# shenwei356/LexicMap

Measured on AMD Instinct MI355X. Metric: queries/sec (lexicmap search hot path, seed index HBM-resident), higher is better.
Workload: dtype u64

## Files before the change

### lexicmap_amd/csrc/lm_algos.h

```cpp
#pragma once
#include <stdint.h>

#if defined(__HIPCC__)
#define LM_HD __host__ __device__ __forceinline__
#define LM_HDN __host__ __device__ inline
#else
#define LM_HD inline
#define LM_HDN inline
#endif

#define LM_NULL_OFF (-1073741824)

LM_HD int lm_clz64(uint64_t x) {
#if defined(__HIP_DEVICE_COMPILE__)
    return x ? __clzll((long long)x) : 64;
#else
    return x ? __builtin_clzll(x) : 64;
#endif
}

LM_HD uint8_t lm_base2bit(uint8_t c) {
    switch (c | 0x20) {
    case 'c': case 'b': case 's': case 'y': return 1;
    case 'g': case 'k': return 2;
// ... 1258 lines not shown
}
LM_HD bool lm_pa_rule_bit(const uint32_t *rule, uint32_t f, int p) {
    const uint32_t p9 = f >> ((p - LM_PFX_BASES2) << 1);
    return (f & ((1u << ((p - 9) << 1)) - 1u)) == 0 && ((rule[p9 >> 5] >> (p9 & 31)) & 1u) != 0;
}
LM_HD bool lm_pa_candidate3(const uint32_t *bloom, int blog, const uint32_t *rule, const uint32_t *bits11, int log,
                            uint32_t f, int p) {
    const uint32_t p11 = f >> ((p - LM_PFX_BASES) << 1);
    const uint32_t a = lm_pa_bloom_slot(p11, 0, blog), b = lm_pa_bloom_slot(p11, 1, blog);
    bool hit = (((bloom[a >> 5] >> (a & 31)) & (bloom[b >> 5] >> (b & 31))) & 1u) != 0;
    if (hit && log > blog) {
        const uint32_t h = lm_pa_filter_slot(p11, log);
        hit = ((bits11[h >> 5] >> (h & 31)) & 1u) != 0;
    }
    return hit || lm_pa_rule_bit(rule, f, p);
}

LM_HD bool lm_tree_search_range_tab(const uint64_t *keys, int n, uint64_t key, int p, int K, const uint32_t *tab,
                                    int tab_bits, int *lo_out, int *hi_out) {
    if (n <= 0) return false;
    if (p > K) p = K;
    const int sh = (K - p) << 1;
    const uint64_t low = sh >= 64 ? ~0ull : ((1ull << sh) - 1);
    const uint64_t left = key & ~low, right = key | low;
    const uint32_t b = (uint32_t)(key >> ((K << 1) - tab_bits));
    int lo = lm_lower_bound_u64(keys, (int)tab[b], (int)tab[b + 1], left);
    int hi = lm_upper_bound_u64(keys, lo, (int)tab[b + 1], right);
    if (lo < hi) {
        *lo_out = lo;
        *hi_out = hi;
// ... 442 lines not shown
```

### lexicmap_amd/csrc/lm_internal.h

```cpp
#pragma once
#include <hip/hip_runtime.h>

#include <algorithm>
#include <atomic>
#include <chrono>
#include <cstdio>
#include <cstdlib>
#include <map>
#include <memory>
#include <deque>
#include <mutex>
#include <shared_mutex>
#include <stdexcept>
#include <string>
#include <unordered_map>
#include <vector>

#include "../../include/lexicmap_hip.h"
#include "lm_format.h"
#include "lm_kernels.h"

namespace lm {

struct HipError : std::runtime_error {
// ... 381 lines not shown
                   unsigned long long *n_out = nullptr);
void lm_screen_capture(lm_index *ix, hipStream_t st, const uint8_t *d_ascii, const std::vector<int64_t> &src_off,
                       const std::vector<int32_t> &len, const std::vector<int32_t> &reg_off, const std::vector<int32_t> &reg_s,
                       const std::vector<int32_t> &reg_e, uint64_t *d_kmers);
}

#define LM_WFA_CLASSES 5
struct lm_tune {
    int wfa_first_nc[LM_WFA_CLASSES] = {2, 2, 4, 8, 8};
    int wfa_win[LM_WFA_CLASSES] = {0, 0, 1, 0, 1};
    int chain1_wave = 1;
    int pa_filter_roll = 1;
    int pa_seg_by_group = 1;
    int pa_drop_nested = 1;
    int pa_rule_map = 1;
    int wfa_resident_pct = 100;
    int arena_reserve_pct = 90;
    int two_lanes = 1;
    int lookup_flat = 1;
    int wfa_r16 = 1;
    int wfa_serial = 0;
    int no_pipeline = 0;
    lm_tune() {
        if (const char *e = getenv("LM_WFA_FIRST_NC")) {
            int v[LM_WFA_CLASSES];
            if (sscanf(e, "%d,%d,%d,%d,%d", &v[0], &v[1], &v[2], &v[3], &v[4]) == LM_WFA_CLASSES)
                for (int c = 0; c < LM_WFA_CLASSES; c++)
                    if (v[c] == 1 || v[c] == 2 || v[c] == 4 || v[c] == 8 || v[c] == 16) wfa_first_nc[c] = v[c];
        }
        if (const char *e = getenv("LM_WFA_WIN"))
            for (int c = 0; c < LM_WFA_CLASSES && e[c]; c++) wfa_win[c] = e[c] == '1';
        if (const char *e = getenv("LM_WFA_R16")) wfa_r16 = atoi(e) != 0;
        if (const char *e = getenv("LM_LOOKUP_FLAT")) lookup_flat = atoi(e) != 0;
        if (const char *e = getenv("LM_CHAIN1_WAVE")) chain1_wave = atoi(e) != 0;
        if (const char *e = getenv("LM_TWO_LANES")) two_lanes = atoi(e) != 0;
        if (const char *e = getenv("LM_ARENA_RESERVE_PCT")) arena_reserve_pct = std::max(0, std::min(100, atoi(e)));
        if (const char *e = getenv("LM_PA_FILTER_ROLL")) pa_filter_roll = atoi(e) != 0;
        if (const char *e = getenv("LM_PA_DROP_NESTED")) pa_drop_nested = atoi(e) != 0;
        if (const char *e = getenv("LM_PA_RULE_MAP")) pa_rule_map = atoi(e) != 0;
    }
};

struct lm_index {
    lm_tune tune;
    int active_lanes = 1;
    int budget_lanes = 1;
    std::mutex mu;
    HostIndex host;
    lm_options opt;
    int device = 0;
    std::string err;
    DBuf<uint64_t> d_masks, d_pk_keys, d_pk_vals, d_out_kmers, d_out_vals, d_g_bg;
    DBuf<uint32_t> d_part_tab, d_g_keep;
    DBuf<int32_t> d_pfx_first, d_g_len, d_g2local;
// ... 56 lines not shown
```

### lexicmap_amd/csrc/lm_kernels.h

```cpp
#pragma once
#include <hip/hip_runtime.h>
#include <stdint.h>

#include "lm_algos.h"
#include "lm_residency.h"

namespace lm {

struct DevIndexView {
    int K, M, mask_prefix;
    const uint64_t *masks;
    const int32_t *pfx_first;
    int part_bases;
    int P1;
    int key_bits;
    int gid_bits, pos_bits;
    const uint64_t *pk_keys;
    const uint64_t *pk_vals;
    const uint32_t *part_tab;
    const int64_t *md_off;
    const uint64_t *g_bg;
    const uint32_t *g_keep;
    const uint64_t *out_kmers;
    const uint64_t *out_vals;
// ... 83 lines not shown
                       float min_score, int32_t *ntask);
void launch_make_tasks(hipStream_t st, DevIndexView ix, const uint64_t *segA, const int64_t *seg_off, int nseg,
                       const LmSub *subs, const int32_t *chain_off_pool, const int32_t *chain_idx_pool,
                       const int32_t *ntask, const int64_t *task_off, const int64_t *qoff, int ext_len,
                       int32_t *order_scratch, Task *tasks);
void launch_task_wlen(hipStream_t st, const Task *tasks, int64_t ntasks, int32_t *wlen);
void launch_task_set_woff(hipStream_t st, Task *tasks, int64_t ntasks, const int64_t *woff);
void launch_extract_windows(hipStream_t st, DevIndexView ix, const Task *tasks, const TaskSrc *src, int64_t ntasks,
                            const int32_t *only, uint8_t *wbuf);
void launch_extract_windows_at(hipStream_t st, DevIndexView ix, const Task *tasks, const TaskSrc *src, const int32_t *idx,
                               const int64_t *dest, int64_t n, uint8_t *wbuf);
void launch_stage_genome_bits(hipStream_t st, const StageCmd *cmds, int64_t n);
void launch_build_cmp_tab(hipStream_t st, const uint64_t *keys_cmp, const int64_t *posoff, const int32_t *nvalid, int nq,
                          int K, const int64_t *tab_off, const int32_t *tab_bits, int64_t tab_words, uint32_t *tab);
void launch_sum_i32(hipStream_t st, const int32_t *v, int64_t n, unsigned long long *out);
void launch_build_cmp_bits(hipStream_t st, const uint64_t *keys_cmp, const int64_t *posoff, const int32_t *nvalid, int nq,
                           int K, const int64_t *bits_off, const int32_t *bits_log, uint32_t *bits);
#define LM_PA_MAX_SEGS 8192
#define LM_PA_RANGE_SEGS 16
#define LM_PA_GROUP 64
void launch_pa_filter(hipStream_t st, DevIndexView ix, const Task *tasks, const TaskSrc *src, int64_t ntasks, const uint8_t *wbuf,
                      const int64_t *posoff, const int32_t *nvalid, const uint32_t *cmp_bits, const int64_t *bits_off,
                      const int32_t *bits_log, int K, int min_prefix, unsigned long long *seg_count, int nseg, int64_t seg_cap,
                      uint64_t *cand, unsigned long long *group_counter, int ncu, int seg_by_group, bool roll = true,
                      bool rule = true);
void launch_pa_search(hipStream_t st, DevIndexView ix, const Task *tasks, const TaskSrc *src, const uint8_t *wbuf, const uint64_t *keys_cmp,
                      const uint32_t *vals_cmp, const int64_t *posoff, const int32_t *nvalid, const uint32_t *cmp_tab,
                      const int64_t *tab_off, const int32_t *tab_bits, int K, int min_prefix,
                      const unsigned long long *seg_count, int nseg, int64_t seg_cap, const uint64_t *cand,
                      unsigned long long *count, int64_t cap, uint64_t *outA, uint64_t *outB, int qbits, int tbits,
                      int xcd_map, bool drop_nested = true);
void launch_pa_task_off_sorted(hipStream_t st, const uint64_t *sortedA, int shift, int64_t total, int64_t ntasks,
                               int64_t *pa_off);
void launch_pa_chain(hipStream_t st, const uint64_t *B, const int64_t *pa_off, int64_t ntasks, int K, LmChain2Opt opt,
                     LmSub *subs, uint8_t *marks, uint64_t *msi, int32_t *stack, LmChain2 *out, int32_t *out_n,
                     int32_t *clr_n, int qbits, int tbits);
void launch_gather_chain2(hipStream_t st, const LmChain2 *in, const int64_t *pa_off, const int32_t *out_n,
                          const int64_t *res_off, int64_t ntasks, LmChain2 *out);
void launch_extend_count(hipStream_t st, const HspIn *hsps, int64_t n, const uint8_t *qseq, const int64_t *qoff,
                         const uint8_t *wbuf, int32_t *cap);
// ... 17 lines not shown
```

### lexicmap_amd/csrc/lm_kernels.hip

```cpp
#include <hip/hip_runtime.h>
#include <stdint.h>

#include <algorithm>

#include "lm_algos.h"
#include "lm_kernels.h"
#include "lm_lookup_dev.h"

namespace lm {

#define LDS_WAVE_SYNC()                                        \
    do {                                                       \
        __builtin_amdgcn_fence(__ATOMIC_RELEASE, "wavefront"); \
        __builtin_amdgcn_wave_barrier();                       \
        __builtin_amdgcn_fence(__ATOMIC_ACQUIRE, "wavefront"); \
    } while (0)

__device__ __forceinline__ int find_segment(const int64_t *off, int n, int64_t x) {
    int lo = 0, hi = n;
    while (lo < hi) {
        int mid = (lo + hi + 1) >> 1;
        if (off[mid] <= x)
            lo = mid;
        else
// ... 62 lines not shown
    for (int64_t t = (int64_t)blockIdx.x * blockDim.x + threadIdx.x; t < total; t += (int64_t)gridDim.x * blockDim.x) {
        const int q = find_segment(tab_off, nq, t);
        const int bits = tab_bits[q], nb = 1 << bits;
        const int b = (int)(t - tab_off[q]);
        const uint64_t *keys = keys_cmp + 2 * posoff[q];
        int n = nvalid[q];
        int lo = n;
        if (b < nb) {
            uint64_t target = (uint64_t)b << ((K << 1) - bits);
            lo = lm_lower_bound_u64(keys, 0, n, target);
        }
        tab[t] = (uint32_t)lo;
    }
}
__global__ __launch_bounds__(256) void k_build_cmp_bits(const uint64_t *__restrict__ keys_cmp,
                                                         const int64_t *__restrict__ posoff,
                                                         const int32_t *__restrict__ nvalid, int nq, int K,
                                                         const int64_t *__restrict__ bits_off,
                                                         const int32_t *__restrict__ bits_log, uint32_t *__restrict__ bits) {
    for (int q = blockIdx.x; q < nq; q += gridDim.x) {
        const uint64_t *keys = keys_cmp + 2 * posoff[q];
        const int n = nvalid[q];
        const int log = bits_log[q];
        uint32_t *b = bits + bits_off[q];
        lm_pa_filter_preset(log, (int)threadIdx.x, (int)blockDim.x, [&](uint64_t w, uint32_t m) { atomicOr(&b[w], m); });
        for (int j = threadIdx.x; j < n; j += blockDim.x)
            lm_pa_filter_set(keys[j], K, log, [&](uint64_t w, uint32_t m) { atomicOr(&b[w], m); });
    }
}

__global__ void k_fill_u32(uint32_t *p, int64_t n, uint32_t v) {
    for (int64_t i = (int64_t)blockIdx.x * blockDim.x + threadIdx.x; i < n; i += (int64_t)gridDim.x * blockDim.x) p[i] = v;
}

__global__ void k_mask(const uint64_t *__restrict__ keys_all, const int64_t *__restrict__ posoff, int nq, int M, int K,
                       const uint64_t *__restrict__ masks, uint64_t *__restrict__ out_kmers,
                       int64_t *__restrict__ out_lo, int64_t *__restrict__ out_hi, uint32_t *__restrict__ first_mask) {
    int64_t total = (int64_t)nq * M;
    for (int64_t t = (int64_t)blockIdx.x * blockDim.x + threadIdx.x; t < total; t += (int64_t)gridDim.x * blockDim.x) {
        int q = (int)(t / M), m = (int)(t % M);
        int64_t base = 2 * posoff[q];
        int n = (int)(2 * (posoff[q + 1] - posoff[q]));
// ... 816 lines not shown
        r = any;
    }
    return r;
}
template <bool ROLL, bool SRC, bool RULE>
__global__ __launch_bounds__(PA_THREADS) void k_pa_filter(DevIndexView ix, const Task *__restrict__ tasks,
                                                           const TaskSrc *__restrict__ src, int64_t ntasks,
                                                           const uint8_t *__restrict__ wbuf,
                                                           const int64_t *__restrict__ posoff,
                                                           const int32_t *__restrict__ nvalid,
                                                           const uint32_t *__restrict__ cmp_bits,
                                                           const int64_t *__restrict__ bits_off,
                                                           const int32_t *__restrict__ bits_log, int K, int min_prefix,
                                                           unsigned long long *__restrict__ seg_count, int nseg,
                                                           int64_t seg_cap, uint64_t *__restrict__ cand,
                                                           unsigned long long *__restrict__ group_counter, int seg_by_group) {
    extern __shared__ uint64_t pa_lds[];
    uint64_t *s_stage = pa_lds;
    uint32_t *s_bloom = (uint32_t *)(pa_lds + PA_WAVES * PA_STAGE);
    uint32_t *s_map9 = s_bloom + (1 << (LM_PA_BLOOM_LOG_MAX - 5));
    uint64_t *s_pend_rec = (uint64_t *)(s_map9 + (1 << (LM_PA_MAP9_LOG - 5)));
    uint32_t *s_pend_pf = (uint32_t *)(s_pend_rec + PA_WAVES * PA_PEND);
    const int tid = threadIdx.x, lane = tid & 63, wave = tid >> 6;
    uint64_t *stg = s_stage + wave * PA_STAGE;
    int n_stg = 0;
    const uint64_t lt_mask = lane ? (~0ull >> (64 - lane)) : 0ull;
    int seg = (int)(((int64_t)blockIdx.x * PA_WAVES + wave) % nseg);
    uint64_t *seg_list = cand + (int64_t)seg * seg_cap;
    auto flush = [&]() {
        if (n_stg == 0) return;
        unsigned long long base = 0;
// ... 3 lines not shown
            if ((int64_t)(base + (unsigned long long)j) < seg_cap) seg_list[base + (unsigned long long)j] = stg[j];
        n_stg = 0;
    };
    auto push = [&](bool c, uint64_t rec) {
        const uint64_t m = __ballot(c);
        if (m == 0) return;
        if (c) stg[n_stg + __popcll(m & lt_mask)] = rec;
        n_stg += __popcll(m);
        if (n_stg > PA_STAGE - 128) flush();
    };
    uint32_t *pend_pf = s_pend_pf + wave * PA_PEND;
    uint64_t *pend_rec = s_pend_rec + wave * PA_PEND;
    int n_pend = 0;
    const uint32_t *cur_qbits = nullptr;
    int cur_log = 0, cur_blog = 0;
    auto pend_round = [&](int cnt) {
        const int idx = n_pend - cnt + lane;
        bool c = false;
        uint64_t rec = 0;
        if (lane < cnt) {
            const uint32_t e = pend_pf[idx];
            rec = pend_rec[idx];
            if constexpr (RULE) {
                const uint32_t h = lm_pa_filter_slot((e & 0x3fffffffu) >> (4 * (int)(e >> 30)), cur_log);
                c = ((cur_qbits[h >> 5] >> (h & 31)) & 1u) != 0;
            } else {
                c = lm_pa_candidate2(s_bloom, cur_blog, s_map9, cur_qbits, cur_log, e & 0x3fffffffu, LM_PFX_BASES + 2 * (int)(e >> 30));
            }
        }
        n_pend -= cnt;
        push(c, rec);
    };
    auto pend = [&](bool c, uint32_t e, uint64_t rec) {
        const uint64_t m = __ballot(c);
        if (m == 0) return;
        if (c) {
            const int slot = n_pend + __popcll(m & lt_mask);
            pend_pf[slot] = e;
            pend_rec[slot] = rec;
        }
// ... 20 lines not shown
    };
    __shared__ int32_t s_q[PA_GROUP], s_rc[PA_GROUP], s_tb[PA_GROUP], s_wlen[PA_GROUP], s_npos[PA_GROUP], s_log[PA_GROUP];
    __shared__ int32_t s_first[PA_GROUP + 1];
    __shared__ int64_t s_goff[PA_GROUP], s_bits[PA_GROUP], s_woff[PA_GROUP];
    __shared__ const uint8_t *s_gb[SRC ? PA_GROUP : 1];
    __shared__ int s_next;
    __shared__ unsigned long long s_grp;
    const int64_t ngroups = (ntasks + PA_GROUP - 1) / PA_GROUP;
    while (true) {
        __syncthreads();
        if (tid == 0) s_grp = atomicAdd(group_counter, 1ull);
        __syncthreads();
        const int64_t grp = (int64_t)s_grp;
        if (grp >= ngroups) break;
        const int64_t t0g = grp * PA_GROUP;
        const int ng = (int)((ntasks < t0g + PA_GROUP ? ntasks : t0g + PA_GROUP) - t0g);
        if (seg_by_group) {
            const int gseg = (int)(grp * (int64_t)(nseg / PA_WAVES) / ngroups) * PA_WAVES + wave;
            if (gseg != seg) {
                flush();
                seg = gseg;
                seg_list = cand + (int64_t)seg * seg_cap;
            }
        }
        __syncthreads();
        if (tid < ng) {
            const Task t = tasks[t0g + tid];
            const int n = nvalid[t.q];
            s_q[tid] = (int32_t)t.q;
            s_rc[tid] = t.rc;
            s_tb[tid] = t.tBegin;
            s_wlen[tid] = t.wlen;
            s_npos[tid] = n > 0 && t.wlen - K + 1 > 0 ? t.wlen - K + 1 : 0;
            if constexpr (SRC) {
                s_gb[tid] = t.g >= 0 ? src[t0g + tid].base : nullptr;
                s_goff[tid] = t.g >= 0 ? src[t0g + tid].off : 0;
            } else {
                s_goff[tid] = t.g >= 0 ? ix.g_off[t.g] : -1;
            }
            s_woff[tid] = t.woff;
            s_bits[tid] = cmp_bits ? bits_off[t.q] : -1;
            s_log[tid] = cmp_bits ? bits_log[t.q] : 0;
        }
        __syncthreads();
        int r0 = 0;
        while (r0 < ng) {
            int r1 = r0 + 1;
            while (r1 < ng && s_q[r1] == s_q[r0]) r1++;
            const int log = s_log[r0], blog = lm_pa_bloom_log(log);
            const uint32_t *qbits = s_bits[r0] >= 0 ? cmp_bits + s_bits[r0] : nullptr;
            cur_qbits = qbits;
            cur_log = log;
            cur_blog = blog;
            if (qbits != nullptr && K >= 16) {
                const uint32_t *gbl = qbits + lm_pa_bloom_word0(log), *g9 = qbits + (RULE ? lm_pa_rule_word0(log) : lm_pa_map9_word0(log));
                const int nb = 1 << (blog - 5);
                for (int j = tid; j < nb; j += PA_THREADS) s_bloom[j] = gbl[j];
// ... 26 lines not shown
                t.tBegin = s_tb[j];
                t.wlen = s_wlen[j];
                const int npos = s_npos[j];
                const int slice = ROLL ? (npos + (s_first[j + 1] - s_first[j]) - 1) / (s_first[j + 1] - s_first[j]) : PA_SLICE;
                const int p0 = (sl - s_first[j]) * slice, p1 = p0 + slice < npos ? p0 + slice : npos;
                const int64_t goff = s_goff[j];
                const uint8_t *gb;
                if constexpr (SRC) gb = s_gb[j];
                else gb = goff >= 0 ? ix.gbits : nullptr;
                const uint8_t *w = wbuf + s_woff[j];
                const int m = pa_min_prefix(min_prefix, t.wlen);
                const int p = m > K ? K : m;
                const bool use_bits = qbits != nullptr && p >= LM_PFX_BASES && K >= LM_PFX_BASES;
                const bool fast_pfx = use_bits && gb != nullptr && p <= 15 && K >= 16;
                const uint64_t rec_t = (uint64_t)(t0g + j) << 32;
                if (ROLL && fast_pfx && K == 31 && p1 > p0) {
                    const int np = p1 - p0;
                    const int bpl = (np + 63) >> 6;
                    const int g0 = t.rc ? t.tBegin + t.wlen - K - (p1 - 1) : t.tBegin + p0;
                    const int64_t abs0 = goff * 4 + g0;
                    const int rl0 = bpl * lane;
                    const int64_t ab = abs0 + (rl0 < np ? rl0 : 0);
                    const uint32_t *gd = (const uint32_t *)gb;
                    const int64_t d0 = ab >> 4, dlast = (abs0 + np + K - 2) >> 4;
                    uint32_t e[5];
#pragma unroll
                    for (int k = 0; k < 5; k++) e[k] = __builtin_bswap32(gd[d0 + k < dlast ? d0 + k : dlast]);
                    const int ob = (int)(ab & 15) * 2;
                    uint32_t S0, S1, S2, S3;
                    {
// ... 23 lines not shown
                            const int r = rl0 + 16 * half + jj;
                            const int i = t.rc ? p1 - 1 - r : p0 + r;
                            const bool in = r < np;
                            bool c0, c1;
                            const uint32_t a0 = pf0 >> sha, a1 = pf1 >> sha;
                            const uint32_t s00 = lm_pa_bloom_slot(a0, 0, blog), s01 = lm_pa_bloom_slot(a0, 1, blog);
                            const uint32_t s10 = lm_pa_bloom_slot(a1, 0, blog), s11 = lm_pa_bloom_slot(a1, 1, blog);
                            const uint32_t b00 = s_bloom[s00 >> 5], b01 = s_bloom[s01 >> 5];
                            const uint32_t b10 = s_bloom[s10 >> 5], b11 = s_bloom[s11 >> 5];
                            const bool h0 = in && (((b00 >> (s00 & 31)) & (b01 >> (s01 & 31))) & 1u) != 0;
                            const bool h1 = in && (((b10 >> (s10 & 31)) & (b11 >> (s11 & 31))) & 1u) != 0;
                            if constexpr (RULE) {
                                const bool r0 = in && lm_pa_rule_bit(s_map9, pf0, p), r1 = in && lm_pa_rule_bit(s_map9, pf1, p);
                                c0 = h0 || r0;
                                c1 = h1 || r1;
                                if (log > blog) {
                                    c0 = r0;
                                    c1 = r1;
                                    pend2(h0 && !r0, h1 && !r1, pf0 | pcode, pf1 | pcode, rec_t | ((uint64_t)(uint32_t)i << 1));
                                }
                            } else {
                                const bool q0 = in && !h0 && (pf0 & m9p) == 0, q1 = in && !h1 && (pf1 & m9p) == 0;
                                c0 = h0;
                                c1 = h1;
                                if (log > blog) {
                                    c0 = c1 = false;
                                    const uint64_t rec = rec_t | ((uint64_t)(uint32_t)i << 1);
                                    pend(h0 || q0, pf0 | pcode, rec);
                                    pend(h1 || q1, pf1 | pcode, rec | 1ull);
                                } else if (__ballot(q0 || q1) != 0ull) {
                                    c0 = pa_partial_rule(q0, c0, pf0, p, blog, s_bloom, s_map9);
// ... 38 lines not shown
                        const bool in = r < np;
                        bool c0, c1;
                        {
                            const uint32_t a0 = pf0 >> ((p - LM_PFX_BASES) << 1), a1 = pf1 >> ((p - LM_PFX_BASES) << 1);
                            const uint32_t s00 = lm_pa_bloom_slot(a0, 0, blog), s01 = lm_pa_bloom_slot(a0, 1, blog);
                            const uint32_t s10 = lm_pa_bloom_slot(a1, 0, blog), s11 = lm_pa_bloom_slot(a1, 1, blog);
                            const uint32_t b00 = s_bloom[s00 >> 5], b01 = s_bloom[s01 >> 5];
                            const uint32_t b10 = s_bloom[s10 >> 5], b11 = s_bloom[s11 >> 5];
                            const bool h0 = in && (((b00 >> (s00 & 31)) & (b01 >> (s01 & 31))) & 1u) != 0;
                            const bool h1 = in && (((b10 >> (s10 & 31)) & (b11 >> (s11 & 31))) & 1u) != 0;
                            if constexpr (RULE) {
                                const bool r0 = in && lm_pa_rule_bit(s_map9, pf0, p), r1 = in && lm_pa_rule_bit(s_map9, pf1, p);
                                const uint32_t pcode = (uint32_t)((p - LM_PFX_BASES) >> 1) << 30;
                                c0 = h0 || r0;
                                c1 = h1 || r1;
                                if (log > blog) {
                                    c0 = r0;
                                    c1 = r1;
                                    pend2(h0 && !r0, h1 && !r1, pf0 | pcode, pf1 | pcode, rec_t | ((uint64_t)(uint32_t)i << 1));
                                }
                            } else {
                                const uint32_t m9p = (1u << ((p - 9) << 1)) - 1u;
                                const bool q0 = in && !h0 && (pf0 & m9p) == 0, q1 = in && !h1 && (pf1 & m9p) == 0;
                                c0 = h0;
                                c1 = h1;
                                if (log > blog) {
                                    c0 = c1 = false;
                                    const uint64_t rec = rec_t | ((uint64_t)(uint32_t)i << 1);
                                    const uint32_t pcode = (uint32_t)((p - LM_PFX_BASES) >> 1) << 30;
                                    pend(h0 || q0, pf0 | pcode, rec);
                                    pend(h1 || q1, pf1 | pcode, rec | 1ull);
// ... 79 lines not shown
        sub = r % blocks_per_seg;
        if (seg >= nseg) return;
    } else {
        seg = blockIdx.x / blocks_per_seg;
        sub = blockIdx.x % blocks_per_seg;
    }
    const uint64_t *cand = cand_all + (int64_t)seg * seg_cap;
    int64_t nc = (int64_t)seg_count[seg];
    if (nc > seg_cap) nc = seg_cap;
    const int sh_t = 2, sh_l = 2 + tbits, sh_q = 8 + tbits, sh_a = 8 + tbits + qbits;
    const uint64_t ccc = lm_ns(1, K), ggg = lm_ns(2, K), ttt = lm_kmer_mask(K);
    const int64_t stride = (int64_t)blocks_per_seg * blockDim.x;
    for (int64_t base = (int64_t)sub * blockDim.x; base < nc; base += stride) {
        const int64_t ci = base + threadIdx.x;
        unsigned long long d_0 = 0, d_1 = 0, d_it = 0, d_an = 0, d_ne = 0;
        if (dbg) d_0 = wall_clock64();
        int j = 0, hi = 0, i = 0;
        int nb = -1, pmin = 0;
        bool rcs = false;
        uint64_t key = 0, right = 0;
        int64_t ti = 0;
        uint32_t qb = 0, qe = 0;
        const uint64_t *keys = nullptr;
        const uint32_t *vals = nullptr;
        if (ci < nc) {
            const uint64_t rec = cand[ci];
            ti = (int64_t)(rec >> 32);
            i = (int)((uint32_t)rec >> 1);
            rcs = (rec & 1ull) != 0;
            const Task t = tasks[ti];
// ... 38 lines not shown
                const uint32_t x = (v & LM_CMP_POS_MASK) >> 1;
                uint32_t pp;
                if (!rcs) {
                    pp = x;
                    if (!((v & 1u) == 1u || pp < qb || pp + lp > qe)) {
                        ok = true;
                        B = lm_pack_anchor((int)pp, (int)lp, i, false, false);
                    }
                } else {
                    pp = x + (uint32_t)K - lp;
                    if (!((v & 1u) == 0u || pp + lp < qb || pp > qe)) {
                        ok = true;
                        B = lm_pack_anchor((int)pp, (int)lp, i + K - (int)lp, true, true);
                    }
                }
                if (ok && lm_pa_nested_match(rcs, K, pmin, (int)lp, nb, v >> LM_CMP_NB_SHIFT, (int)pp, (int)qb)) {
                    if (dbg) d_ne++;
                    if (drop_nested) ok = false;
                }
                j++;
            }
            const uint64_t m = __ballot(ok);
            if (m) {
                if (ok) {
                    if (qbits > 0) {
                        const LmSub u = lm_unpack_anchor(B);
                        B = ((uint64_t)ti << sh_a) | ((uint64_t)(uint32_t)u.qbegin << sh_q) |
                            ((uint64_t)(32 - (int)u.len) << sh_l) | ((uint64_t)(uint32_t)u.tbegin << sh_t) |
                            ((uint64_t)u.qrc << 1) | (uint64_t)u.trc;
                    }
                    const int slot = n_stg + __popcll(m & lt_mask);
                    stg[slot] = B;
                    stt[slot] = (uint32_t)ti;
                }
                n_stg += __popcll(m);
                d_an += (unsigned long long)__popcll(m);
                if (n_stg > PAS_STAGE - 64) flush();
            }
        }
        if (dbg) {
            const unsigned long long nc_w = (unsigned long long)__popcll(__ballot(ci < nc)), d_2 = wall_clock64();
            for (int o = 32; o > 0; o >>= 1) d_ne += __shfl_xor(d_ne, o, 64);
            if (lane == 0) {
                atomicAdd(dbg + 0, nc_w);
                atomicAdd(dbg + 1, 1ull);
                atomicAdd(dbg + 2, d_it);
                atomicAdd(dbg + 3, d_an);
                atomicAdd(dbg + 4, d_1 - d_0);
                atomicAdd(dbg + 5, d_2 - d_1);
                atomicAdd(dbg + 6, d_ne);
            }
        }
    }
    flush();
}
__global__ void k_pa_task_off_sorted(const uint64_t *__restrict__ sortedA, int shift, int64_t total, int64_t ntasks,
                                     int64_t *__restrict__ pa_off) {
    for (int64_t i = (int64_t)blockIdx.x * blockDim.x + threadIdx.x; i <= ntasks; i += (int64_t)gridDim.x * blockDim.x) {
        int64_t lo = 0, hi = total;
        while (lo < hi) {
            int64_t mid = (lo + hi) >> 1;
            if ((sortedA[mid] >> shift) < (uint64_t)i)
                lo = mid + 1;
            else
                hi = mid;
// ... 949 lines not shown
                       n, wbuf);
}
void launch_stage_genome_bits(hipStream_t st, const StageCmd *cmds, int64_t n) {
    if (n <= 0) return;
    hipLaunchKernelGGL(k_stage_genome_bits, dim3((unsigned)std::min<int64_t>(n, 65536)), dim3(256), 0, st, cmds, n);
}
void launch_build_cmp_tab(hipStream_t st, const uint64_t *keys_cmp, const int64_t *posoff, const int32_t *nvalid, int nq,
                          int K, const int64_t *tab_off, const int32_t *tab_bits, int64_t tab_words, uint32_t *tab) {
    LM_LAUNCH_1D(k_build_cmp_tab, tab_words, st, keys_cmp, posoff, nvalid, nq, K, tab_off, tab_bits, tab);
}
void launch_sum_i32(hipStream_t st, const int32_t *v, int64_t n, unsigned long long *out) {
    int g = (int)((n + 255) / 256);
    g = g < 1 ? 1 : (g > 2048 ? 2048 : g);
    hipLaunchKernelGGL(k_sum_i32, dim3(g), dim3(256), 0, st, v, n, out);
}
void launch_build_cmp_bits(hipStream_t st, const uint64_t *keys_cmp, const int64_t *posoff, const int32_t *nvalid, int nq,
                           int K, const int64_t *bits_off, const int32_t *bits_log, uint32_t *bits) {
    int g = nq < 1 ? 1 : (nq > 65536 ? 65536 : nq);
    hipLaunchKernelGGL(k_build_cmp_bits, dim3(g), dim3(256), 0, st, keys_cmp, posoff, nvalid, nq, K, bits_off, bits_log, bits);
}
static decltype(&k_pa_filter<true, true, true>) pa_filter_kernel(bool roll, bool src, bool rule) {
    if (rule) return src ? (roll ? k_pa_filter<true, true, true> : k_pa_filter<false, true, true>) : (roll ? k_pa_filter<true, false, true> : k_pa_filter<false, false, true>);
    return src ? (roll ? k_pa_filter<true, true, false> : k_pa_filter<false, true, false>) : (roll ? k_pa_filter<true, false, false> : k_pa_filter<false, false, false>);
}
void launch_pa_filter(hipStream_t st, DevIndexView ix, const Task *tasks, const TaskSrc *src, int64_t ntasks, const uint8_t *wbuf,
                      const int64_t *posoff, const int32_t *nvalid, const uint32_t *cmp_bits, const int64_t *bits_off,
                      const int32_t *bits_log, int K, int min_prefix, unsigned long long *seg_count, int nseg, int64_t seg_cap,
                      uint64_t *cand, unsigned long long *group_counter, int ncu, int seg_by_group, bool roll, bool rule) {
    const int64_t ngroups = (ntasks + PA_GROUP - 1) / PA_GROUP;
    int g = (int)(ngroups < 1 ? 1 : (ngroups > ncu ? ncu : ngroups));
    static bool lds_set = false;
    if (!lds_set) {
        for (int v = 0; v < 8; v++) (void)hipFuncSetAttribute((const void *)pa_filter_kernel(v & 1, v & 2, v & 4), hipFuncAttributeMaxDynamicSharedMemorySize, PA_LDS_BYTES);
        lds_set = true;
    }
    roll = roll && K == 31;
    auto kern = pa_filter_kernel(roll, src != nullptr, rule);
    hipLaunchKernelGGL(kern, dim3(g), dim3(PA_THREADS), PA_LDS_BYTES, st, ix, tasks, src, ntasks, wbuf,
                       posoff, nvalid, cmp_bits, bits_off, bits_log, K, min_prefix, seg_count, nseg, seg_cap, cand, group_counter,
                       seg_by_group);
}
void launch_pa_search(hipStream_t st, DevIndexView ix, const Task *tasks, const TaskSrc *src, const uint8_t *wbuf, const uint64_t *keys_cmp,
                      const uint32_t *vals_cmp, const int64_t *posoff, const int32_t *nvalid, const uint32_t *cmp_tab,
                      const int64_t *tab_off, const int32_t *tab_bits, int K, int min_prefix,
                      const unsigned long long *seg_count, int nseg, int64_t seg_cap, const uint64_t *cand,
                      unsigned long long *count, int64_t cap, uint64_t *outA, uint64_t *outB, int qbits, int tbits,
                      int xcd_map, bool drop_nested) {
    int bps = xcd_map ? 256 / LM_PA_RANGE_SEGS : (256 * 32 + nseg - 1) / nseg;
    const int64_t need = (seg_cap + 255) / 256;
    if (bps > need) bps = (int)(need < 1 ? 1 : need);
    const int nseg8 = xcd_map ? (nseg / LM_PA_RANGE_SEGS + 7) / 8 * 8 * LM_PA_RANGE_SEGS : nseg;
    static const bool ps_dbg = getenv("LM_DEBUG_PA_SEARCH") != nullptr;
    static unsigned long long *d_dbg = nullptr;
    if (ps_dbg && !d_dbg && hipMalloc((void **)&d_dbg, 8 * sizeof(unsigned long long)) != hipSuccess) d_dbg = nullptr;
    if (ps_dbg && d_dbg) (void)hipMemsetAsync(d_dbg, 0, 8 * sizeof(unsigned long long), st);
    hipLaunchKernelGGL(src ? k_pa_search<true> : k_pa_search<false>, dim3(nseg8 * bps), dim3(256), 0, st, ix, tasks, src, wbuf, keys_cmp, vals_cmp, posoff, nvalid, cmp_tab,
                       tab_off, tab_bits, K, min_prefix, seg_count, seg_cap, bps, cand, count, cap, outA, outB, qbits, tbits, nseg,
                       xcd_map, drop_nested ? 1 : 0, ps_dbg ? d_dbg : nullptr);
    if (ps_dbg && d_dbg) {
        unsigned long long h[8] = {0};
        (void)hipStreamSynchronize(st);
        (void)hipMemcpy(h, d_dbg, sizeof h, hipMemcpyDeviceToHost);
        const unsigned long long found = h[3] + (drop_nested ? h[6] : 0ull);
        fprintf(stderr, "[lm] k_pa_search: %llu candidates in %llu wavefront passes (%.1f per pass), %llu enumeration passes, %llu anchors (%.2f per enumeration pass), wavefront-ms: search %.1f, enumeration %.1f; %llu anchors found, %llu nested in their neighbour's (%.1f %%, %s)\n",
                h[0], h[1], h[1] ? (double)h[0] / (double)h[1] : 0.0, h[2], h[3], h[2] ? (double)h[3] / (double)h[2] : 0.0, (double)h[4] / 1e5, (double)h[5] / 1e5,
                found, h[6], found ? 100.0 * (double)h[6] / (double)found : 0.0, drop_nested ? "not emitted" : "emitted");
    }
}
void launch_pa_task_off_sorted(hipStream_t st, const uint64_t *sortedA, int shift, int64_t total, int64_t ntasks,
                               int64_t *pa_off) {
    LM_LAUNCH_1D(k_pa_task_off_sorted, ntasks + 1, st, sortedA, shift, total, ntasks, pa_off);
}
void launch_pa_chain(hipStream_t st, const uint64_t *B, const int64_t *pa_off, int64_t ntasks, int K, LmChain2Opt opt,
                     LmSub *subs, uint8_t *marks, uint64_t *msi, int32_t *stack, LmChain2 *out, int32_t *out_n,
                     int32_t *clr_n, int qbits, int tbits) {
    int g = (int)(ntasks < 1 ? 1 : (ntasks > 262144 ? 262144 : ntasks));
    static const bool pa_dbg = getenv("LM_DEBUG_PA_CHAIN") != nullptr;
    static unsigned long long *d_pa_dbg = nullptr;
    if (pa_dbg && !d_pa_dbg && hipMalloc((void **)&d_pa_dbg, 20 * sizeof(unsigned long long)) != hipSuccess) d_pa_dbg = nullptr;
    unsigned long long *dbg = pa_dbg ? d_pa_dbg : nullptr;
    if (dbg) (void)hipMemsetAsync(dbg, 0, 20 * sizeof(unsigned long long), st);
// ... 74 lines not shown
```

### lexicmap_amd/csrc/lm_pipeline.hip

```cpp
#include <hip/hip_runtime.h>

#include <algorithm>
#include <chrono>
#include <cmath>
#include <cstdio>
#include <cstdlib>
#include <malloc.h>
#include <cstring>
#include <map>
#include <mutex>
#include <optional>
#include <sys/stat.h>
#include <stdexcept>
#include <tuple>
#include <string>
#include <unordered_map>
#include <vector>

#include "../../include/lexicmap_hip.h"
#include "lm_format.h"
#include "lm_kernels.h"

#include "lm_internal.h"
#include "lm_prims.h"
// ... 533 lines not shown
            prim_segmented_sort_pairs(S(ix), TMP(ix), w.keys_all.p, w.keys_all2.p, w.vals_all.p, w.vals_all2.p, (size_t)(2 * P),
                                      (size_t)qb->nq, qb->d_segoff.p, 0, end_bit);
        if (PC > 0)
            prim_segmented_sort_pairs(S(ix), TMP(ix), w.keys_cmp.p, w.keys_cmp2.p, w.vals_cmp.p, w.vals_cmp2.p, (size_t)(2 * PC),
                                      (size_t)qb->nq, qb->segoff_cmp(), 0, 64);
    }
    w.k_all = w.keys_all2.p;
    w.v_all = w.vals_all2.p;
    w.k_cmp = w.keys_cmp2.p;
    w.v_cmp = w.vals_cmp2.p;
    w.cmp_tab.ensure((size_t)qb->tab_words + 1);
    launch_build_cmp_tab(S(ix), w.k_cmp, qb->posoff_cmp(), w.nvalid.p, qb->nq, LM_CMP_K, qb->d_tab_off.p, qb->d_tab_bits.p,
                         qb->tab_words, w.cmp_tab.p);
    w.cmp_bits.ensure((size_t)qb->bits_words + 1);
    HIPCHK(hipMemsetAsync(w.cmp_bits.p, 0, (size_t)qb->bits_words * sizeof(uint32_t), S(ix)));
    launch_build_cmp_bits(S(ix), w.k_cmp, qb->posoff_cmp(), w.nvalid.p, qb->nq, LM_CMP_K, qb->d_bits_off.p, qb->d_bits_log.p,
                          w.cmp_bits.p);
}

static void stage_mask(Work &w) {
    lm_index *ix = w.ix;
    lm_qbatch *qb = w.qb;
    int M = ix->host.M;
    int64_t nqm = (int64_t)qb->nq * M;
    w.kmers.ensure((size_t)nqm + 1);
    w.klo.ensure((size_t)nqm + 1);
    w.khi.ensure((size_t)nqm + 1);
    w.first_mask.ensure((size_t)std::max<int64_t>(2 * qb->total_pos, 1));
    launch_fill_u32(S(ix), w.first_mask.p, 2 * qb->total_pos, 0xffffffffu);
    Prof p(ix, "k_mask", nqm * 32);
    launch_mask(S(ix), w.k_all, qb->d_posoff.p, qb->nq, M, ix->host.k, ix->view.masks, w.kmers.p, w.klo.p, w.khi.p,
// ... 887 lines not shown
            h2d(ix, qb->d_posoff_cmp, qb->h_posoff_cmp);
            h2d(ix, qb->d_segoff_cmp, segoff_cmp);
        }
        const std::vector<int64_t> &pc = qb->cmp_split ? qb->h_posoff_cmp : qb->h_posoff;
        h2d(ix, qb->d_seq, qb->h_seq);
        h2d(ix, qb->d_qoff, qb->h_qoff);
        h2d(ix, qb->d_posoff, qb->h_posoff);
        h2d(ix, qb->d_segoff, segoff);
        {
            std::vector<int64_t> boff(nq + 1, 0);
            std::vector<int32_t> blog(nq + 1, 13);
            for (size_t i = 0; i < nq; i++) {
                const int64_t nk = 2 * (pc[i + 1] - pc[i]);
                const int lg = lm_pa_filter_log(nk);
                blog[i] = lg;
                boff[i + 1] = boff[i] + (int64_t)lm_pa_bits_words(lg);
            }
            qb->bits_words = boff[nq];
            std::vector<int64_t> toff(nq + 1, 0);
            std::vector<int32_t> tbits(nq + 1, LM_TAB_BITS_MIN);
            for (size_t i = 0; i < nq; i++) {
                const int64_t nk = 2 * (pc[i + 1] - pc[i]);
                const int tb = lm_cmp_tab_bits(nk);
                tbits[i] = tb;
                toff[i + 1] = toff[i] + ((int64_t)1 << tb) + 1;
            }
            qb->tab_words = toff[nq];
            h2d(ix, qb->d_tab_off, toff);
            h2d(ix, qb->d_tab_bits, tbits);
            h2d(ix, qb->d_bits_off, boff);
            h2d(ix, qb->d_bits_log, blog);
// ... 28 lines not shown
    try {
        std::lock_guard<std::mutex> lock(ix->mu);
        HIPCHK(hipSetDevice(ix->device));
        int64_t max_pos, max_qm;
        part_limits(ix, &max_pos, &max_qm);
        const int K = ix->host.k, M = ix->host.M;
        std::vector<size_t> cuts{0};
        int64_t pos = 0, nqp = 0;
        for (size_t i = 0; i < nq; i++) {
            const int64_t np = std::max<int64_t>((int64_t)queries[i].len - K + 1, 0);
            if (np > max_pos) {
                ix->err = "a query of " + std::to_string(queries[i].len) + " bases exceeds what one pass can hold (" +
                          std::to_string(max_pos) + " k-mers)";
                return LM_ERR_ARG;
            }
            const int64_t per_q = (int64_t)M + (2 * ((int64_t)1 << (LM_PA_MAP9_LOG - 3)) + 79) / 80;
            if (nqp > 0 && (pos + np > max_pos || (nqp + 1) * per_q > max_qm)) {
                cuts.push_back(i);
                pos = 0;
                nqp = 0;
            }
            pos += np;
            nqp++;
        }
        cuts.push_back(nq);
        if (cuts.size() == 2) {
            *out = upload_part(ix, queries, nq, 0);
            return LM_OK;
        }
        lm_qbatch *top = new lm_qbatch();
        top->ix = ix;
// ... 252 lines not shown
            if (attempt == 0 || nseg_stale) nseg = (int)std::max<int64_t>(1, std::min<int64_t>(1024, a.pa_cap / 4096));
            nseg_stale = false;
        } else if (attempt == 0) {
            const int64_t ngroups = (nt + LM_PA_GROUP - 1) / LM_PA_GROUP;
            const int64_t ranges = std::max<int64_t>(1, std::min<int64_t>(std::min<int64_t>(LM_PA_MAX_SEGS / LM_PA_RANGE_SEGS, ngroups),
                                                                          a.pa_cap / 4096 / LM_PA_RANGE_SEGS));
            nseg = (int)ranges * LM_PA_RANGE_SEGS;
        }
        const int64_t seg_cap = a.pa_cap / nseg;
        HIPCHK(hipMemsetAsync(a.pa_count.p, 0, (size_t)(2 + nseg) * sizeof(unsigned long long), S(ix)));
        {
            Prof p(ix, "k_pa_filter", W);
            launch_pa_filter(S(ix), ix->view, tasks_d, src_d, nt, a.wb, qb->posoff_cmp(), a.w->nvalid.p, a.w->cmp_bits.p,
                             qb->d_bits_off.p, qb->d_bits_log.p, LM_CMP_K, 11, a.pa_count.p + 2, nseg, seg_cap, a.B1.p,
                             a.pa_count.p + 1, device_cus(ix->device), by_group ? 1 : 0, ix->tune.pa_filter_roll != 0,
                             ix->tune.pa_rule_map != 0);
        }
        {
            Prof p(ix, "k_pa_search");
            launch_pa_search(S(ix), ix->view, tasks_d, src_d, a.wb, a.w->k_cmp, a.w->v_cmp, qb->posoff_cmp(), a.w->nvalid.p,
                             a.w->cmp_tab.p, qb->d_tab_off.p, qb->d_tab_bits.p, LM_CMP_K, 11, a.pa_count.p + 2, nseg, seg_cap,
                             a.B1.p, a.pa_count.p, a.pa_cap, a.A0.p, a.B0.p, compact ? qbits : 0, compact ? tbits : 0,
                             by_group ? 1 : 0, ix->tune.pa_drop_nested != 0);
        }
        std::vector<unsigned long long> hv((size_t)2 + nseg);
        HIPCHK(hipMemcpyAsync(hv.data(), a.pa_count.p, hv.size() * sizeof(unsigned long long), hipMemcpyDeviceToHost, S(ix)));
        sync(ix);
        TP = (int64_t)hv[0];
        int64_t ncand = 0, seg_max = 0;
        for (int j = 0; j < nseg; j++) {
            ncand += (int64_t)hv[2 + j];
// ... 2335 lines not shown
```

Before: 1409.

## Add per-position-segment prefix bitmaps to narrow pseudo-alignment candidate filtering

Adds a per-query set of positional segment bitmaps (one 2^17-bit filter per 4096 query positions) built alongside the existing prefix filter. In the pa_filter kernel, tasks whose query range spans few segments check only those segments' bits, so fewer false candidates reach the costly pa_search stage. The price is extra bitmap memory and build atomics, an LDS array per group, more deferred pending rounds, and a changed per-query memory budget. A debug counter for candidates without anchors is also added.

```diff
diff --git a/lexicmap_amd/csrc/lm_algos.h b/lexicmap_amd/csrc/lm_algos.h
--- a/lexicmap_amd/csrc/lm_algos.h
+++ b/lexicmap_amd/csrc/lm_algos.h
@@ -1296,6 +1296,53 @@
         hit = ((bits11[h >> 5] >> (h & 31)) & 1u) != 0;
     }
     return hit || lm_pa_rule_bit(rule, f, p);
+}
+
+#define LM_PA_SEG_LOG 12
+#define LM_PA_SEG_BITS_LOG 17
+#define LM_PA_SEG_MAX 3
+LM_HD int lm_pa_nsegs(int64_t npos) { return npos > 0 ? (int)((npos + ((int64_t)1 << LM_PA_SEG_LOG) - 1) >> LM_PA_SEG_LOG) : 0; }
+LM_HD uint64_t lm_pa_seg_word0(int log) { return lm_pa_bits_words(log); }
+LM_HD uint64_t lm_pa_bits_words_seg(int log, int64_t npos) {
+    return lm_pa_bits_words(log) + ((uint64_t)lm_pa_nsegs(npos) << (LM_PA_SEG_BITS_LOG - 5));
+}
+LM_HD uint32_t lm_pa_seg_slot(uint32_t p11) { return lm_pa_filter_slot(p11, LM_PA_SEG_BITS_LOG); }
+template <typename OrBit> LM_HD void lm_pa_filter_set(uint64_t key, uint32_t pos, int K, int log, OrBit or_bit) {
+    lm_pa_filter_set(key, K, log, or_bit);
+    const uint32_t h = lm_pa_seg_slot((uint32_t)(key >> ((K - LM_PFX_BASES) << 1)));
+    or_bit(lm_pa_seg_word0(log) + ((uint64_t)(pos >> LM_PA_SEG_LOG) << (LM_PA_SEG_BITS_LOG - 5)) + (h >> 5), 1u << (h & 31));
+}
+LM_HD bool lm_pa_range_segs(int64_t qbegin, int64_t qend, int K, int64_t npos, int *s0, int *s1) {
+    int64_t lo = qbegin - K, hi = qend + K;
+    if (lo < 0) lo = 0;
+    if (hi > npos - 1) hi = npos - 1;
+    if (hi < lo) return false;
+    const int a = (int)(lo >> LM_PA_SEG_LOG), b = (int)(hi >> LM_PA_SEG_LOG), n = b - a + 1;
+    if (n > LM_PA_SEG_MAX || 2 * n > lm_pa_nsegs(npos)) return false;
+    *s0 = a;
+    *s1 = b;
+    return true;
+}
+LM_HD bool lm_pa_seg_hit(const uint32_t *segs, int s0, int s1, uint32_t p11) {
+    const uint32_t h = lm_pa_seg_slot(p11);
+    bool hit = false;
+    for (int s = s0; s <= s1; s++) hit = hit || ((segs[((uint64_t)s << (LM_PA_SEG_BITS_LOG - 5)) + (h >> 5)] >> (h & 31)) & 1u) != 0;
+    return hit;
+}
+LM_HD bool lm_pa_candidate4(const uint32_t *bloom, int blog, const uint32_t *rule, const uint32_t *bits11, int log,
+                            const uint32_t *segs, int64_t npos, int64_t qbegin, int64_t qend, int K, uint32_t f, int p) {
+    int s0 = 0, s1 = 0;
+    if (!lm_pa_range_segs(qbegin, qend, K, npos, &s0, &s1)) return lm_pa_candidate3(bloom, blog, rule, bits11, log, f, p);
+    if (lm_pa_rule_bit(rule, f, p)) return true;
+    const uint32_t p11 = f >> ((p - LM_PFX_BASES) << 1);
+    const uint32_t a = lm_pa_bloom_slot(p11, 0, blog), b = lm_pa_bloom_slot(p11, 1, blog);
+    if ((((bloom[a >> 5] >> (a & 31)) & (bloom[b >> 5] >> (b & 31))) & 1u) == 0) return false;
+    if (!lm_pa_seg_hit(segs, s0, s1, p11)) return false;
+    if (log > blog) {
+        const uint32_t h = lm_pa_filter_slot(p11, log);
+        return ((bits11[h >> 5] >> (h & 31)) & 1u) != 0;
+    }
+    return true;
 }
 
 LM_HD bool lm_tree_search_range_tab(const uint64_t *keys, int n, uint64_t key, int p, int K, const uint32_t *tab,
diff --git a/lexicmap_amd/csrc/lm_internal.h b/lexicmap_amd/csrc/lm_internal.h
--- a/lexicmap_amd/csrc/lm_internal.h
+++ b/lexicmap_amd/csrc/lm_internal.h
@@ -419,6 +419,7 @@
     int pa_seg_by_group = 1;
     int pa_drop_nested = 1;
     int pa_rule_map = 1;
+    int pa_range_bits = 1;
     int wfa_resident_pct = 100;
     int arena_reserve_pct = 90;
     int two_lanes = 1;
@@ -443,6 +444,7 @@
         if (const char *e = getenv("LM_PA_FILTER_ROLL")) pa_filter_roll = atoi(e) != 0;
         if (const char *e = getenv("LM_PA_DROP_NESTED")) pa_drop_nested = atoi(e) != 0;
         if (const char *e = getenv("LM_PA_RULE_MAP")) pa_rule_map = atoi(e) != 0;
+        if (const char *e = getenv("LM_PA_RANGE_BITS")) pa_range_bits = atoi(e) != 0;
     }
 };
 
diff --git a/lexicmap_amd/csrc/lm_kernels.h b/lexicmap_amd/csrc/lm_kernels.h
--- a/lexicmap_amd/csrc/lm_kernels.h
+++ b/lexicmap_amd/csrc/lm_kernels.h
@@ -121,8 +121,8 @@
 void launch_build_cmp_tab(hipStream_t st, const uint64_t *keys_cmp, const int64_t *posoff, const int32_t *nvalid, int nq,
                           int K, const int64_t *tab_off, const int32_t *tab_bits, int64_t tab_words, uint32_t *tab);
 void launch_sum_i32(hipStream_t st, const int32_t *v, int64_t n, unsigned long long *out);
-void launch_build_cmp_bits(hipStream_t st, const uint64_t *keys_cmp, const int64_t *posoff, const int32_t *nvalid, int nq,
-                           int K, const int64_t *bits_off, const int32_t *bits_log, uint32_t *bits);
+void launch_build_cmp_bits(hipStream_t st, const uint64_t *keys_cmp, const uint32_t *vals_cmp, const int64_t *posoff,
+                           const int32_t *nvalid, int nq, int K, const int64_t *bits_off, const int32_t *bits_log, uint32_t *bits);
 #define LM_PA_MAX_SEGS 8192
 #define LM_PA_RANGE_SEGS 16
 #define LM_PA_GROUP 64
@@ -130,7 +130,7 @@
                       const int64_t *posoff, const int32_t *nvalid, const uint32_t *cmp_bits, const int64_t *bits_off,
                       const int32_t *bits_log, int K, int min_prefix, unsigned long long *seg_count, int nseg, int64_t seg_cap,
                       uint64_t *cand, unsigned long long *group_counter, int ncu, int seg_by_group, bool roll = true,
-                      bool rule = true);
+                      bool rule = true, bool range_bits = true);
 void launch_pa_search(hipStream_t st, DevIndexView ix, const Task *tasks, const TaskSrc *src, const uint8_t *wbuf, const uint64_t *keys_cmp,
                       const uint32_t *vals_cmp, const int64_t *posoff, const int32_t *nvalid, const uint32_t *cmp_tab,
                       const int64_t *tab_off, const int32_t *tab_bits, int K, int min_prefix,
diff --git a/lexicmap_amd/csrc/lm_kernels.hip b/lexicmap_amd/csrc/lm_kernels.hip
--- a/lexicmap_amd/csrc/lm_kernels.hip
+++ b/lexicmap_amd/csrc/lm_kernels.hip
@@ -100,18 +100,20 @@
     }
 }
 __global__ __launch_bounds__(256) void k_build_cmp_bits(const uint64_t *__restrict__ keys_cmp,
+                                                         const uint32_t *__restrict__ vals_cmp,
                                                          const int64_t *__restrict__ posoff,
                                                          const int32_t *__restrict__ nvalid, int nq, int K,
                                                          const int64_t *__restrict__ bits_off,
                                                          const int32_t *__restrict__ bits_log, uint32_t *__restrict__ bits) {
     for (int q = blockIdx.x; q < nq; q += gridDim.x) {
         const uint64_t *keys = keys_cmp + 2 * posoff[q];
+        const uint32_t *vals = vals_cmp + 2 * posoff[q];
         const int n = nvalid[q];
         const int log = bits_log[q];
         uint32_t *b = bits + bits_off[q];
         lm_pa_filter_preset(log, (int)threadIdx.x, (int)blockDim.x, [&](uint64_t w, uint32_t m) { atomicOr(&b[w], m); });
         for (int j = threadIdx.x; j < n; j += blockDim.x)
-            lm_pa_filter_set(keys[j], K, log, [&](uint64_t w, uint32_t m) { atomicOr(&b[w], m); });
+            lm_pa_filter_set(keys[j], (vals[j] & LM_CMP_POS_MASK) >> 1, K, log, [&](uint64_t w, uint32_t m) { atomicOr(&b[w], m); });
     }
 }
 
@@ -958,7 +960,8 @@
                                                            const int32_t *__restrict__ bits_log, int K, int min_prefix,
                                                            unsigned long long *__restrict__ seg_count, int nseg,
                                                            int64_t seg_cap, uint64_t *__restrict__ cand,
-                                                           unsigned long long *__restrict__ group_counter, int seg_by_group) {
+                                                           unsigned long long *__restrict__ group_counter, int seg_by_group,
+                                                           int range_bits) {
     extern __shared__ uint64_t pa_lds[];
     uint64_t *s_stage = pa_lds;
     uint32_t *s_bloom = (uint32_t *)(pa_lds + PA_WAVES * PA_STAGE);
@@ -992,6 +995,8 @@
     int n_pend = 0;
     const uint32_t *cur_qbits = nullptr;
     int cur_log = 0, cur_blog = 0;
+    int64_t cur_t0 = 0;
+    __shared__ int32_t s_seg[PA_GROUP];
     auto pend_round = [&](int cnt) {
         const int idx = n_pend - cnt + lane;
         bool c = false;
@@ -1000,8 +1005,13 @@
             const uint32_t e = pend_pf[idx];
             rec = pend_rec[idx];
             if constexpr (RULE) {
-                const uint32_t h = lm_pa_filter_slot((e & 0x3fffffffu) >> (4 * (int)(e >> 30)), cur_log);
-                c = ((cur_qbits[h >> 5] >> (h & 31)) & 1u) != 0;
+                const uint32_t p11 = (e & 0x3fffffffu) >> (4 * (int)(e >> 30));
+                const int sg = s_seg[(int)((int64_t)(rec >> 32) - cur_t0)];
+                c = sg < 0 || lm_pa_seg_hit(cur_qbits + lm_pa_seg_word0(cur_log), sg >> 2, (sg >> 2) + (sg & 3), p11);
+                if (c && cur_log > cur_blog) {
+                    const uint32_t h = lm_pa_filter_slot(p11, cur_log);
+                    c = ((cur_qbits[h >> 5] >> (h & 31)) & 1u) != 0;
+                }
             } else {
                 c = lm_pa_candidate2(s_bloom, cur_blog, s_map9, cur_qbits, cur_log, e & 0x3fffffffu, LM_PFX_BASES + 2 * (int)(e >> 30));
             }
@@ -1052,6 +1062,7 @@
         const int64_t grp = (int64_t)s_grp;
         if (grp >= ngroups) break;
         const int64_t t0g = grp * PA_GROUP;
+        cur_t0 = t0g;
         const int ng = (int)((ntasks < t0g + PA_GROUP ? ntasks : t0g + PA_GROUP) - t0g);
         if (seg_by_group) {
             const int gseg = (int)(grp * (int64_t)(nseg / PA_WAVES) / ngroups) * PA_WAVES + wave;
@@ -1079,6 +1090,10 @@
             s_woff[tid] = t.woff;
             s_bits[tid] = cmp_bits ? bits_off[t.q] : -1;
             s_log[tid] = cmp_bits ? bits_log[t.q] : 0;
+            int sg0 = 0, sg1 = 0;
+            const bool narrow = RULE && range_bits && cmp_bits &&
+                                lm_pa_range_segs(t.qBegin, t.qEnd, K, posoff[t.q + 1] - posoff[t.q], &sg0, &sg1);
+            s_seg[tid] = narrow ? (sg0 << 2) | (sg1 - sg0) : -1;
         }
         __syncthreads();
         int r0 = 0;
@@ -1135,6 +1150,7 @@
                 const bool use_bits = qbits != nullptr && p >= LM_PFX_BASES && K >= LM_PFX_BASES;
                 const bool fast_pfx = use_bits && gb != nullptr && p <= 15 && K >= 16;
                 const uint64_t rec_t = (uint64_t)(t0g + j) << 32;
+                const bool queue = log > blog || s_seg[j] >= 0;
                 if (ROLL && fast_pfx && K == 31 && p1 > p0) {
                     const int np = p1 - p0;
                     const int bpl = (np + 63) >> 6;
@@ -1188,7 +1204,7 @@
                                 const bool r0 = in && lm_pa_rule_bit(s_map9, pf0, p), r1 = in && lm_pa_rule_bit(s_map9, pf1, p);
                                 c0 = h0 || r0;
                                 c1 = h1 || r1;
-                                if (log > blog) {
+                                if (queue) {
                                     c0 = r0;
                                     c1 = r1;
                                     pend2(h0 && !r0, h1 && !r1, pf0 | pcode, pf1 | pcode, rec_t | ((uint64_t)(uint32_t)i << 1));
@@ -1257,7 +1273,7 @@
                                 const uint32_t pcode = (uint32_t)((p - LM_PFX_BASES) >> 1) << 30;
                                 c0 = h0 || r0;
                                 c1 = h1 || r1;
-                                if (log > blog) {
+                                if (queue) {
                                     c0 = r0;
                                     c1 = r1;
                                     pend2(h0 && !r0, h1 && !r1, pf0 | pcode, pf1 | pcode, rec_t | ((uint64_t)(uint32_t)i << 1));
@@ -1367,6 +1383,7 @@
     for (int64_t base = (int64_t)sub * blockDim.x; base < nc; base += stride) {
         const int64_t ci = base + threadIdx.x;
         unsigned long long d_0 = 0, d_1 = 0, d_it = 0, d_an = 0, d_ne = 0;
+        bool d_any = false;
         if (dbg) d_0 = wall_clock64();
         int j = 0, hi = 0, i = 0;
         int nb = -1, pmin = 0;
@@ -1435,6 +1452,7 @@
                         B = lm_pack_anchor((int)pp, (int)lp, i + K - (int)lp, true, true);
                     }
                 }
+                if (dbg && ok) d_any = true;
                 if (ok && lm_pa_nested_match(rcs, K, pmin, (int)lp, nb, v >> LM_CMP_NB_SHIFT, (int)pp, (int)qb)) {
                     if (dbg) d_ne++;
                     if (drop_nested) ok = false;
@@ -1461,6 +1479,7 @@
         }
         if (dbg) {
             const unsigned long long nc_w = (unsigned long long)__popcll(__ballot(ci < nc)), d_2 = wall_clock64();
+            const unsigned long long ne_w = (unsigned long long)__popcll(__ballot(ci < nc && !d_any));
             for (int o = 32; o > 0; o >>= 1) d_ne += __shfl_xor(d_ne, o, 64);
             if (lane == 0) {
                 atomicAdd(dbg + 0, nc_w);
@@ -1470,6 +1489,7 @@
                 atomicAdd(dbg + 4, d_1 - d_0);
                 atomicAdd(dbg + 5, d_2 - d_1);
                 atomicAdd(dbg + 6, d_ne);
+                atomicAdd(dbg + 7, ne_w);
             }
         }
     }
@@ -2449,10 +2469,10 @@
     g = g < 1 ? 1 : (g > 2048 ? 2048 : g);
     hipLaunchKernelGGL(k_sum_i32, dim3(g), dim3(256), 0, st, v, n, out);
 }
-void launch_build_cmp_bits(hipStream_t st, const uint64_t *keys_cmp, const int64_t *posoff, const int32_t *nvalid, int nq,
-                           int K, const int64_t *bits_off, const int32_t *bits_log, uint32_t *bits) {
+void launch_build_cmp_bits(hipStream_t st, const uint64_t *keys_cmp, const uint32_t *vals_cmp, const int64_t *posoff,
+                           const int32_t *nvalid, int nq, int K, const int64_t *bits_off, const int32_t *bits_log, uint32_t *bits) {
     int g = nq < 1 ? 1 : (nq > 65536 ? 65536 : nq);
-    hipLaunchKernelGGL(k_build_cmp_bits, dim3(g), dim3(256), 0, st, keys_cmp, posoff, nvalid, nq, K, bits_off, bits_log, bits);
+    hipLaunchKernelGGL(k_build_cmp_bits, dim3(g), dim3(256), 0, st, keys_cmp, vals_cmp, posoff, nvalid, nq, K, bits_off, bits_log, bits);
 }
 static decltype(&k_pa_filter<true, true, true>) pa_filter_kernel(bool roll, bool src, bool rule) {
     if (rule) return src ? (roll ? k_pa_filter<true, true, true> : k_pa_filter<false, true, true>) : (roll ? k_pa_filter<true, false, true> : k_pa_filter<false, false, true>);
@@ -2461,7 +2481,8 @@
 void launch_pa_filter(hipStream_t st, DevIndexView ix, const Task *tasks, const TaskSrc *src, int64_t ntasks, const uint8_t *wbuf,
                       const int64_t *posoff, const int32_t *nvalid, const uint32_t *cmp_bits, const int64_t *bits_off,
                       const int32_t *bits_log, int K, int min_prefix, unsigned long long *seg_count, int nseg, int64_t seg_cap,
-                      uint64_t *cand, unsigned long long *group_counter, int ncu, int seg_by_group, bool roll, bool rule) {
+                      uint64_t *cand, unsigned long long *group_counter, int ncu, int seg_by_group, bool roll, bool rule,
+                      bool range_bits) {
     const int64_t ngroups = (ntasks + PA_GROUP - 1) / PA_GROUP;
     int g = (int)(ngroups < 1 ? 1 : (ngroups > ncu ? ncu : ngroups));
     static bool lds_set = false;
@@ -2473,7 +2494,7 @@
     auto kern = pa_filter_kernel(roll, src != nullptr, rule);
     hipLaunchKernelGGL(kern, dim3(g), dim3(PA_THREADS), PA_LDS_BYTES, st, ix, tasks, src, ntasks, wbuf,
                        posoff, nvalid, cmp_bits, bits_off, bits_log, K, min_prefix, seg_count, nseg, seg_cap, cand, group_counter,
-                       seg_by_group);
+                       seg_by_group, range_bits && rule ? 1 : 0);
 }
 void launch_pa_search(hipStream_t st, DevIndexView ix, const Task *tasks, const TaskSrc *src, const uint8_t *wbuf, const uint64_t *keys_cmp,
                       const uint32_t *vals_cmp, const int64_t *posoff, const int32_t *nvalid, const uint32_t *cmp_tab,
@@ -2497,9 +2518,10 @@
         (void)hipStreamSynchronize(st);
         (void)hipMemcpy(h, d_dbg, sizeof h, hipMemcpyDeviceToHost);
         const unsigned long long found = h[3] + (drop_nested ? h[6] : 0ull);
-        fprintf(stderr, "[lm] k_pa_search: %llu candidates in %llu wavefront passes (%.1f per pass), %llu enumeration passes, %llu anchors (%.2f per enumeration pass), wavefront-ms: search %.1f, enumeration %.1f; %llu anchors found, %llu nested in their neighbour's (%.1f %%, %s)\n",
+        fprintf(stderr, "[lm] k_pa_search: %llu candidates in %llu wavefront passes (%.1f per pass), %llu enumeration passes, %llu anchors (%.2f per enumeration pass), wavefront-ms: search %.1f, enumeration %.1f; %llu anchors found, %llu nested in their neighbour's (%.1f %%, %s); %llu candidates without an anchor before that rule (%.1f %%)\n",
                 h[0], h[1], h[1] ? (double)h[0] / (double)h[1] : 0.0, h[2], h[3], h[2] ? (double)h[3] / (double)h[2] : 0.0, (double)h[4] / 1e5, (double)h[5] / 1e5,
-                found, h[6], found ? 100.0 * (double)h[6] / (double)found : 0.0, drop_nested ? "not emitted" : "emitted");
+                found, h[6], found ? 100.0 * (double)h[6] / (double)found : 0.0, drop_nested ? "not emitted" : "emitted", h[7],
+                h[0] ? 100.0 * (double)h[7] / (double)h[0] : 0.0);
     }
 }
 void launch_pa_task_off_sorted(hipStream_t st, const uint64_t *sortedA, int shift, int64_t total, int64_t ntasks,
diff --git a/lexicmap_amd/csrc/lm_pipeline.hip b/lexicmap_amd/csrc/lm_pipeline.hip
--- a/lexicmap_amd/csrc/lm_pipeline.hip
+++ b/lexicmap_amd/csrc/lm_pipeline.hip
@@ -571,7 +571,7 @@
                          qb->tab_words, w.cmp_tab.p);
     w.cmp_bits.ensure((size_t)qb->bits_words + 1);
     HIPCHK(hipMemsetAsync(w.cmp_bits.p, 0, (size_t)qb->bits_words * sizeof(uint32_t), S(ix)));
-    launch_build_cmp_bits(S(ix), w.k_cmp, qb->posoff_cmp(), w.nvalid.p, qb->nq, LM_CMP_K, qb->d_bits_off.p, qb->d_bits_log.p,
+    launch_build_cmp_bits(S(ix), w.k_cmp, w.v_cmp, qb->posoff_cmp(), w.nvalid.p, qb->nq, LM_CMP_K, qb->d_bits_off.p, qb->d_bits_log.p,
                           w.cmp_bits.p);
 }
 
@@ -1489,7 +1489,7 @@
                 const int64_t nk = 2 * (pc[i + 1] - pc[i]);
                 const int lg = lm_pa_filter_log(nk);
                 blog[i] = lg;
-                boff[i + 1] = boff[i] + (int64_t)lm_pa_bits_words(lg);
+                boff[i + 1] = boff[i] + (int64_t)lm_pa_bits_words_seg(lg, pc[i + 1] - pc[i]);
             }
             qb->bits_words = boff[nq];
             std::vector<int64_t> toff(nq + 1, 0);
@@ -1548,7 +1548,7 @@
                           std::to_string(max_pos) + " k-mers)";
                 return LM_ERR_ARG;
             }
-            const int64_t per_q = (int64_t)M + (2 * ((int64_t)1 << (LM_PA_MAP9_LOG - 3)) + 79) / 80;
+            const int64_t per_q = (int64_t)M + (2 * ((int64_t)1 << (LM_PA_MAP9_LOG - 3)) + ((int64_t)1 << (LM_PA_SEG_BITS_LOG - 3)) + 79) / 80;
             if (nqp > 0 && (pos + np > max_pos || (nqp + 1) * per_q > max_qm)) {
                 cuts.push_back(i);
                 pos = 0;
@@ -1831,7 +1831,7 @@
             launch_pa_filter(S(ix), ix->view, tasks_d, src_d, nt, a.wb, qb->posoff_cmp(), a.w->nvalid.p, a.w->cmp_bits.p,
                              qb->d_bits_off.p, qb->d_bits_log.p, LM_CMP_K, 11, a.pa_count.p + 2, nseg, seg_cap, a.B1.p,
                              a.pa_count.p + 1, device_cus(ix->device), by_group ? 1 : 0, ix->tune.pa_filter_roll != 0,
-                             ix->tune.pa_rule_map != 0);
+                             ix->tune.pa_rule_map != 0, ix->tune.pa_range_bits != 0);
         }
         {
             Prof p(ix, "k_pa_search");
```

Result: no change. 1432 (median of 6 runs) (+1.6%).
